# lmb-freiburg/hand3d

Hardware: NVIDIA H100
Metric: images/sec full pipeline 320x320 (higher is better)
Workload: dtype bf16 hi/lo split x3 MMA passes, fp32 accumulate (fp32 parity, 1e-3)

## Files before the change

### hand3d_b200/csrc/common.cuh

```cuda
#pragma once
#include <cuda_runtime.h>
#include <cuda_bf16.h>
#include <cuda_fp16.h>
#include <stdint.h>
#include <stdio.h>
#include <algorithm>
#include <cmath>
#include <string>

#include "../../include/hand3d_b200.h"

namespace h3d {

void set_error(const char* fmt, ...);
int cuda_fail(cudaError_t e, const char* what, const char* file, int line);

#define H3D_CUDA(expr)                                                     \
    do {                                                                   \
        cudaError_t _e = (expr);                                           \
        if (_e != cudaSuccess) return h3d::cuda_fail(_e, #expr, __FILE__, __LINE__); \
    } while (0)

#define H3D_CHECK_LAUNCH() H3D_CUDA(cudaGetLastError())

// ... 165 lines not shown
              int out_f, int leaky, int x_stride, cudaStream_t s);
int launch_concat_handside(const float* feat, const float* hand_side, float* out, int B, int feat_n, cudaStream_t s);
int launch_concat_handside_split(const float* feat, const float* hand_side, Split out, int B, int feat_n, int Kpad, Half16 t, cudaStream_t s);

int launch_conv_c3_tc(const float* x, const float* w, const float* bias, Split y, int Cs_total, int cs_off, int B, int H, int W, int leaky,
                      Half16 half, cudaStream_t s, int* err_flag = nullptr, const int* count = nullptr, const int* slots = nullptr);
struct TcConvPlan;
struct TcConvDesc {
    Split x;
    int Cin_total, Cin_pad;
    Split w;
    const float* bias;
    const float* w_scale = nullptr;
    int Cout, Cout_pad;
    Split y;
    int Cy_total, cy_off;
    float* yf;
    int Cyf_total, cyf_off;
    int B, H, W, k, leaky;
    int passes;
    float corr_scale = 0.f;
    Half16 half;
    int pool = 0;
    int* err_flag = nullptr;
    const int* count = nullptr;
};
struct TcTuning {
    int bn = 0;
    int chunk_kb = 0;
    int no_side_stream = 0, no_pool_fusion = 0, lift_direct = 0;
    int c3_ffma = 0;
    int no_seg_fusion = 0;
    int fc_chain = 1;
    int pdl = 1;
};
TcTuning& tc_tuning();
int tc_set_tuning(const char* key, int value);
struct FcLayerDesc {
    Split x; int x_stride, in_features;
    Split w; const float* bias; int out_features, out_pad;
    const float* w_scale = nullptr;
    Split y; int y_stride;
    float* yf; int yf_stride;
    int leaky;
};
struct FcChainDesc { FcLayerDesc layer[4]; int num_layers = 0; };
struct FcChainPlan;
FcChainPlan* fc_chain_plan_create(const FcChainDesc* chains, int num_chains, int B, Half16 half, const float* can, const float* uxyz,
                                  unsigned int* counter, int* err_flag);
void fc_chain_plan_destroy(FcChainPlan* p);
int fc_chain_launch(const FcChainPlan* p, const float* hand_side, float* rot, float* out, cudaStream_t s);
TcConvPlan* tc_conv_plan_create(const TcConvDesc& d, int* rc = nullptr);
void tc_conv_plan_destroy(TcConvPlan* p);
int tc_conv_launch(const TcConvPlan* p, cudaStream_t s);
int64_t tc_conv_flops(const TcConvPlan* p);
int tc_num_sms();
void tc_conv_geometry(int B, int H, int W, int Cout_pad, int pool, int passes, int out[4]);

int launch_pack_conv_w(const float* w_hwio, const float* bias, Split out, float* bias_pad, float* w_scale, int k, int Cin, int Cout,
                       int Cin_pad, int Cout_pad, bool dgrad, Half16 half, cudaStream_t s);
int conv_grad_prep_blocks(int64_t pixels, int64_t* pixels_per_block);
int launch_conv_grad_prep(const float* dy, const float* y, Split out, float* db_part, int B, int H, int W, int Cout, int Cout_pad,
                          int stride, int leaky, cudaStream_t s);
int launch_bias_grad_reduce(const float* db_part, int nblk, int Cout, int Cout_pad, float* db, cudaStream_t s);
struct WgradDesc {
    Split x;
// ... 39 lines not shown
```

### hand3d_b200/csrc/conv_wgmma.cu

```cuda
#include <cuda.h>

#include <algorithm>
#include <cstdlib>
#include <cstring>
#include <vector>

#include "common.cuh"
#include "split_fmt.cuh"
#include "wgmma_common.cuh"

namespace h3d {

namespace {

constexpr int BM = 128;
constexpr int BK = 64;
constexpr int kThreads = 384;
constexpr int kConsumerThreads = 256;
constexpr int A_TILE_BYTES = BM * BK * 2;
constexpr int STG_COLS = 64;
constexpr int STG_PITCH = STG_COLS + 1;
constexpr int STG_BYTES = BM * STG_PITCH * 4;
constexpr int kSmemBudget = 227 * 1024 - 2048 - STG_BYTES;

__host__ __device__ constexpr int stage_bytes(int BN, int PASSES) { return (PASSES >= 3 ? 2 : 1) * (A_TILE_BYTES + BN * BK * 2); }
__host__ __device__ constexpr int num_stages(int BN, int PASSES) {
    return kSmemBudget / stage_bytes(BN, PASSES) > 8 ? 8 : kSmemBudget / stage_bytes(BN, PASSES);
}
__host__ __device__ constexpr int smem_bytes(int BN, int PASSES) { return num_stages(BN, PASSES) * stage_bytes(BN, PASSES) + STG_BYTES + 2048; }

struct TcParams {
    const float* bias;
    uint16_t* y_hi; uint16_t* y_lo; uint8_t* y_l8; uint8_t* y_h8; int Cy_total, cy_off;
    float corr_scale;
    float* yf; int Cyf_total, cyf_off;
    int B, H, W, k, pad, cin_chunks;
    int TW, TH, TB, tiles_w, tiles_h, n_tiles, num_tiles;
    int n_valid;
    int pool;
    int chunk_kb;
    int leaky;
    int* err_flag;
    const float* w_scale;
    const int* count;
};

__device__ __forceinline__ int counted_images(const TcParams& p) { return p.count ? min(*p.count, p.B) : p.B; }
__device__ __forceinline__ int counted_tiles(const TcParams& p, int nb) {
    return p.count ? min(p.num_tiles, (nb + p.TB - 1) / p.TB * p.tiles_w * p.tiles_h * p.n_tiles) : p.num_tiles;
}

template <int PASSES, bool FP16, bool SMEM_SCALE = false>
__device__ __forceinline__ void epilogue_store32(const TcParams& p, const float* a, int64_t pix, int n, bool valid, const float* w_scale) {
    float f[32];
    const float4* bp = reinterpret_cast<const float4*>(p.bias + n);
#pragma unroll
    for (int q = 0; q < 8; ++q) {
        const float4 bv = __ldg(bp + q);
        if (PASSES == 4) {
            f[4 * q + 0] = fmaf(a[4 * q + 0], p.corr_scale, bv.x);
            f[4 * q + 1] = fmaf(a[4 * q + 1], p.corr_scale, bv.y);
            f[4 * q + 2] = fmaf(a[4 * q + 2], p.corr_scale, bv.z);
            f[4 * q + 3] = fmaf(a[4 * q + 3], p.corr_scale, bv.w);
        } else if (FP16) {
            const float4 sv = SMEM_SCALE ? reinterpret_cast<const float4*>(w_scale + n)[q] : __ldg(reinterpret_cast<const float4*>(w_scale + n) + q);
            f[4 * q + 0] = fmaf(a[4 * q + 0], sv.x, bv.x);
            f[4 * q + 1] = fmaf(a[4 * q + 1], sv.y, bv.y);
            f[4 * q + 2] = fmaf(a[4 * q + 2], sv.z, bv.z);
            f[4 * q + 3] = fmaf(a[4 * q + 3], sv.w, bv.w);
        } else {
            f[4 * q + 0] = a[4 * q + 0] + bv.x;
            f[4 * q + 1] = a[4 * q + 1] + bv.y;
            f[4 * q + 2] = a[4 * q + 2] + bv.z;
            f[4 * q + 3] = a[4 * q + 3] + bv.w;
        }
    }
    if (p.leaky) {
#pragma unroll
        for (int q = 0; q < 32; ++q) f[q] = fmaxf(f[q], kNegSlope * f[q]);
    }
    if (p.pool == 1) {
#pragma unroll
        for (int q = 0; q < 32; ++q) {
            f[q] = fmaxf(f[q], __shfl_xor_sync(0xFFFFFFFFu, f[q], 1));
            f[q] = fmaxf(f[q], __shfl_xor_sync(0xFFFFFFFFu, f[q], p.TW));
        }
    }
    if (!valid) return;
    if (n + 32 > p.n_valid) {
        const int cnt = p.n_valid - n;
        if (p.yf && cnt > 0) {
            float* dst = p.yf + pix * p.Cyf_total + p.cyf_off + n;
#pragma unroll
            for (int q = 0; q < 32; ++q)
                if (q < cnt) dst[q] = f[q];
        }
#pragma unroll
        for (int q = 0; q < 32; ++q)
            if (q >= cnt) f[q] = 0.f;
    } else if (p.yf) {
        if (((p.Cyf_total | p.cyf_off) & 3) == 0) {
            float4* dst = reinterpret_cast<float4*>(p.yf + pix * p.Cyf_total + p.cyf_off + n);
#pragma unroll
            for (int q = 0; q < 8; ++q) dst[q] = make_float4(f[4 * q], f[4 * q + 1], f[4 * q + 2], f[4 * q + 3]);
        } else {
            float* dst = p.yf + pix * p.Cyf_total + p.cyf_off + n;
#pragma unroll
            for (int q = 0; q < 32; ++q) dst[q] = f[q];
        }
    }
    if (p.y_hi) {
        const int64_t off = pix * p.Cy_total + p.cy_off + n;
        uint4* dh = reinterpret_cast<uint4*>(p.y_hi + off);
        uint4* dl = reinterpret_cast<uint4*>(p.y_lo + off);
#pragma unroll
        for (int g = 0; g < 4; ++g) {
            uint32_t hi[4], lo[4];
#pragma unroll
// ... 113 lines not shown
                for (int j = 0; j < 2; ++j) {
                    const uint64_t koff = (uint64_t)j * 2;
                    mma8<BN>(acc8, a_l8 + koff, b_h8 + koff, (uint32_t)((kb > kb0) | (j != 0)));
                    mma8<BN>(acc8, a_h8 + koff, b_l8 + koff, 1u);
                }
            }
            wgmma_commit();
            fence_regs<NR>(acc);
            fence_regs<NR8>(acc8);
            H3D_SKEW(SKEW_COMMIT, kb);
            wgmma_wait<1>();
            if (pend >= 0 && lane == 0) mbar_arrive(&r.empty[pend]);
            pend = r.stage;
            if (++r.stage == C::STAGES) { r.stage = 0; r.phase ^= 1; }
        }
        wgmma_wait<0>();
        if (lane == 0) mbar_arrive(&r.empty[pend]);
        fence_regs<NR>(acc);
        fence_regs<NR8>(acc8);
        if constexpr (PASSES == 4) {
#pragma unroll
            for (int i = 0; i < NR; ++i) acc[i] += acc8[i];
        }
        if (kb0 == 0) {
#pragma unroll
            for (int i = 0; i < NR; ++i) racc[i] = acc[i];
        } else {
#pragma unroll
            for (int i = 0; i < NR; ++i) racc[i] += acc[i];
        }
    }
}

template <int BN, int PASSES, bool FP16, class PixOf, bool SMEM_SCALE = false>
__device__ __forceinline__ void store_tile(const TcParams& p, const float* racc, float* stg, int ct, int n0, PixOf pix_of,
                                           const float* w_scale) {
    const int wg = ct >> 7, tt = ct & 127;
    const int r0 = wg * 64 + (tt >> 5) * 16 + ((tt & 31) >> 2);
    const int cq = 2 * (tt & 3);
    const int row = ct & 127, half = ct >> 7;
    int64_t pix; bool valid;
    pix_of(row, pix, valid);
#pragma unroll
    for (int rnd = 0; rnd < BN / STG_COLS; ++rnd) {
        H3D_SKEW(SKEW_EPILOGUE, 2 * rnd);
        named_bar_sync(1, kConsumerThreads);
#pragma unroll
        for (int j = 0; j < STG_COLS / 8; ++j) {
            const int jj = rnd * (STG_COLS / 8) + j, c = 8 * j + cq;
            stg[r0 * STG_PITCH + c] = racc[4 * jj];
            stg[r0 * STG_PITCH + c + 1] = racc[4 * jj + 1];
            stg[(r0 + 8) * STG_PITCH + c] = racc[4 * jj + 2];
            stg[(r0 + 8) * STG_PITCH + c + 1] = racc[4 * jj + 3];
        }
        named_bar_sync(1, kConsumerThreads);
        H3D_SKEW(SKEW_EPILOGUE, 2 * rnd + 1);
        float f[32];
#pragma unroll
        for (int q = 0; q < 32; ++q) f[q] = stg[row * STG_PITCH + half * 32 + q];
        epilogue_store32<PASSES, FP16, SMEM_SCALE>(p, f, pix, n0 + rnd * STG_COLS + half * 32, valid, w_scale);
    }
}

constexpr int kProducerRegs = 40, kConsumerRegs = 232;

template <int BN, int PASSES, bool FP16>
__global__ void __launch_bounds__(kThreads, 1)
conv_tc_kernel(const __grid_constant__ CUtensorMap map_x_hi, const __grid_constant__ CUtensorMap map_x_lo,
               const __grid_constant__ CUtensorMap map_w_hi, const __grid_constant__ CUtensorMap map_w_lo,
               const __grid_constant__ CUtensorMap map_x_h8, const __grid_constant__ CUtensorMap map_w_l8, const TcParams p) {
    using C = RingCfg<BN, PASSES>;
    static_assert(PASSES != 4 || FP16, "fp8-correction mode uses an fp16 main plane");
    static_assert(smem_bytes(BN, PASSES) <= 227 * 1024, "conv_tc_kernel: shared memory budget");

    extern __shared__ __align__(1024) uint8_t smem_raw[];
    uint8_t* smem = reinterpret_cast<uint8_t*>((reinterpret_cast<uintptr_t>(smem_raw) + 1023) & ~(uintptr_t)1023);
    float* stg = reinterpret_cast<float*>(smem + C::STAGES * C::STAGE_BYTES);
    uint64_t* bars = reinterpret_cast<uint64_t*>(smem + C::STAGES * C::STAGE_BYTES + STG_BYTES);
    Ring ring{smem, bars, bars + C::STAGES, 0, 0};

    const int warp = threadIdx.x >> 5, lane = threadIdx.x & 31;
    const int wg = __shfl_sync(0xFFFFFFFFu, (int)threadIdx.x / 128, 0);
    const int kblocks = p.k * p.k * p.cin_chunks;

    if (threadIdx.x == 0) {
        prefetch_tmap(&map_x_hi); prefetch_tmap(&map_w_hi);
        if (PASSES >= 3) { prefetch_tmap(&map_x_lo); prefetch_tmap(&map_w_lo); }
        if (PASSES == 4) { prefetch_tmap(&map_x_h8); prefetch_tmap(&map_w_l8); }
        for (int s = 0; s < C::STAGES; ++s) { mbar_init(&ring.full[s], 1); mbar_init(&ring.empty[s], kConsumerThreads / 32); }
        asm volatile("fence.mbarrier_init.release.cluster;" ::: "memory");
    }
    __syncthreads();
    pdl_launch_dependents();
    H3D_SKEW(SKEW_PDL_TAIL, 0);
    pdl_wait();
    const int nb = counted_images(p), num_tiles = counted_tiles(p, nb);

    if (wg == 0) {
        setmaxnreg_dec<kProducerRegs>();
        if (warp == 0) {
            for (int tile = blockIdx.x; tile < num_tiles; tile += gridDim.x) {
                const int nt = tile % p.n_tiles, mt = tile / p.n_tiles;
                const int tw = mt % p.tiles_w, th = (mt / p.tiles_w) % p.tiles_h, tb = mt / (p.tiles_w * p.tiles_h);
                const int w0 = tw * p.TW - p.pad, h0 = th * p.TH - p.pad, b0 = tb * p.TB, n0 = nt * BN;
                int kcol = 0;
                for (int kh = 0; kh < p.k; ++kh)
                    for (int kw = 0; kw < p.k; ++kw)
                        for (int cc = 0; cc < p.cin_chunks; ++cc, kcol += BK)
                            produce_kblock<BN, PASSES>(ring, &map_x_hi, &map_x_lo, &map_x_h8, &map_w_hi, &map_w_lo, &map_w_l8, cc * BK,
                                                       w0 + kw, h0 + kh, b0, kcol, n0, p.err_flag);
            }
        }
    } else {
        setmaxnreg_inc<kConsumerRegs>();
        const int ct = threadIdx.x - 128;
        float racc[BN / 2];
        for (int tile = blockIdx.x; tile < num_tiles; tile += gridDim.x) {
            const int nt = tile % p.n_tiles, mt = tile / p.n_tiles;
            const int tw = mt % p.tiles_w, th = (mt / p.tiles_w) % p.tiles_h, tb = mt / (p.tiles_w * p.tiles_h);
            mma_tile<BN, PASSES, FP16>(ring, kblocks, p.chunk_kb, racc, ct >> 7, lane, p.err_flag);
            store_tile<BN, PASSES, FP16>(p, racc, stg, ct, nt * BN, [&](int row, int64_t& pix, bool& valid) {
                const int w_l = row % p.TW, h_l = (row / p.TW) % p.TH, b_l = row / (p.TW * p.TH);
                const int w = tw * p.TW + w_l, h = th * p.TH + h_l, b = tb * p.TB + b_l;
                valid = (w < p.W) && (h < p.H) && (b < nb);
                pix = ((int64_t)b * p.H + h) * p.W + w;
                if (p.pool) {
                    const int par = p.pool == 2 ? 1 : 0;
                    valid = valid && ((w & 1) == par) && ((h & 1) == par);
                    pix = ((int64_t)b * (p.H >> 1) + (h >> 1)) * (p.W >> 1) + (w >> 1);
                }
            }, p.w_scale);
        }
    }
}

constexpr int C3_TW = 16, C3_TH = 8;
constexpr int C3T_THREADS = 256;
constexpr int C3T_B_BYTES = 128 * BK * 2;
constexpr int C3T_PW = C3_TW + 2, C3T_PH = C3_TH + 2;
constexpr int C3T_PATCH_FLOATS = C3T_PH * C3T_PW * 3;
constexpr int C3T_SMEM = C3T_B_BYTES + 2 * A_TILE_BYTES + STG_BYTES + C3T_PATCH_FLOATS * 4 + 64 * 4 + 1024 ;

template <bool FP16, bool COUNTED>
__global__ void __launch_bounds__(C3T_THREADS, 2)
conv_c3_tc_kernel(const float* __restrict__ x, const float* __restrict__ w, const TcParams p, const int* __restrict__ slots) {
    extern __shared__ __align__(1024) uint8_t smem_raw[];
    uint8_t* smem = reinterpret_cast<uint8_t*>((reinterpret_cast<uintptr_t>(smem_raw) + 1023) & ~(uintptr_t)1023);
    uint8_t* bsm = smem;
    uint8_t* asm_ = smem + C3T_B_BYTES;
    float* stg = reinterpret_cast<float*>(asm_ + 2 * A_TILE_BYTES);
    float* patch = stg + BM * STG_PITCH;
    float* w_scale = patch + C3T_PATCH_FLOATS;

    const int t = threadIdx.x, wg = t >> 7;
    if (t < 128) {
        const int co = t & 63;
        int sh = 0;
        if (FP16) {
            float mx = 0.f;
            for (int k = 0; k < 27; ++k) mx = fmaxf(mx, fabsf(__ldg(w + k * 64 + co)));
            sh = fp16_w_shift(mx);
            if (t < 64) w_scale[co] = ldexpf(1.f, -sh);
        }
        uint32_t pk[16];
// ... 223 lines not shown
                    box, estr, CU_TENSOR_MAP_INTERLEAVE_NONE, es == 2 ? CU_TENSOR_MAP_SWIZZLE_128B : CU_TENSOR_MAP_SWIZZLE_64B,
                    CU_TENSOR_MAP_L2_PROMOTION_L2_256B, CU_TENSOR_MAP_FLOAT_OOB_FILL_NONE);
    if (r != CUDA_SUCCESS) { set_error("cuTensorMapEncodeTiled(activations) failed: %d", (int)r); return false; }
    return true;
}

bool encode_w_map(CUtensorMap* m, const void* base, int Ktot, int Cout_pad, int BN, int es) {
    EncodeTiledFn fn = get_encode_fn();
    if (!fn) return false;
    cuuint64_t dims[2] = {(cuuint64_t)Ktot, (cuuint64_t)Cout_pad};
    cuuint64_t strides[1] = {(cuuint64_t)Ktot * es};
    cuuint32_t box[2] = {(cuuint32_t)BK, (cuuint32_t)BN};
    cuuint32_t estr[2] = {1, 1};
    CUresult r = fn(m, es == 2 ? CU_TENSOR_MAP_DATA_TYPE_UINT16 : CU_TENSOR_MAP_DATA_TYPE_UINT8, 2, const_cast<void*>(base), dims, strides,
                    box, estr, CU_TENSOR_MAP_INTERLEAVE_NONE, es == 2 ? CU_TENSOR_MAP_SWIZZLE_128B : CU_TENSOR_MAP_SWIZZLE_64B,
                    CU_TENSOR_MAP_L2_PROMOTION_L2_256B, CU_TENSOR_MAP_FLOAT_OOB_FILL_NONE);
    if (r != CUDA_SUCCESS) { set_error("cuTensorMapEncodeTiled(weights) failed: %d", (int)r); return false; }
    return true;
}

namespace {

void choose_tile(int B, int H, int W, int* TW, int* TH, int* TB, bool pool = false) {
    static const int cand[][3] = {{16, 8, 1}, {8, 16, 1}, {32, 4, 1}, {4, 32, 1}, {64, 2, 1}, {128, 1, 1}, {8, 8, 2},
                                  {16, 4, 2}, {4, 16, 2}, {8, 4, 4}, {4, 8, 4}, {4, 4, 8}, {8, 2, 8}, {2, 2, 32}, {1, 1, 128}};
    int64_t best = -1;
    for (auto& c : cand) {
        if (pool && !((c[0] % 2) == 0 && c[0] <= 16 && (c[1] % 2) == 0)) continue;
        const int64_t tiles = (int64_t)ceil_div(W, c[0]) * ceil_div(H, c[1]) * ceil_div(B, c[2]);
        if (best < 0 || tiles < best) { best = tiles; *TW = c[0]; *TH = c[1]; *TB = c[2]; }
    }
}

template <int BN, int PASSES, bool FP16>
int launch_inst(const TcConvPlan* pl, cudaStream_t s);

}

struct TcConvPlan {
    int device = 0;
    TcConvDesc d;
    CUtensorMap map_x_hi, map_x_lo, map_w_hi, map_w_lo, map_x_h8, map_w_l8;
    TcParams p;
    int BN, grid;
};

constexpr int kMaxDevices = 64;
static int current_device() { int dev = 0; if (cudaGetDevice(&dev) != cudaSuccess) { cudaGetLastError(); dev = 0; } return dev; }
int tc_num_sms() {
    static int n[kMaxDevices] = {};
    const int dev = current_device() % kMaxDevices;
    if (!n[dev]) {
        int v = 0;
        if (cudaDeviceGetAttribute(&v, cudaDevAttrMultiProcessorCount, dev) != cudaSuccess || v <= 0) { cudaGetLastError(); v = 132; }
        n[dev] = v;
    }
    return n[dev];
}
template <typename K>
static int smem_opt_in(K kernel, int bytes, bool* done ) {
    const int dev = current_device() % kMaxDevices;
    if (!done[dev]) {
        H3D_CUDA(cudaFuncSetAttribute(kernel, cudaFuncAttributeMaxDynamicSharedMemorySize, bytes));
        done[dev] = true;
    }
    return H3D_OK;
}

template <typename... KArgs, typename... Args>
static cudaError_t launch_pdl(void (*kernel)(KArgs...), dim3 grid, dim3 block, size_t smem, cudaStream_t s, Args&&... args) {
    cudaLaunchConfig_t cfg = {};
    cfg.gridDim = grid; cfg.blockDim = block; cfg.dynamicSmemBytes = smem; cfg.stream = s;
    cudaLaunchAttribute attr[1];
    attr[0].id = cudaLaunchAttributeProgrammaticStreamSerialization;
    attr[0].val.programmaticStreamSerializationAllowed = tc_tuning().pdl ? 1 : 0;
    cfg.attrs = attr; cfg.numAttrs = 1;
    return cudaLaunchKernelEx(&cfg, kernel, static_cast<KArgs>(args)...);
}

TcTuning& tc_tuning() {
    static TcTuning t = [] {
        TcTuning v;
        auto geti = [](const char* n, int d) { const char* e = getenv(n); return e ? atoi(e) : d; };
        v.bn = geti("H3D_TC_BN", 0);
        v.chunk_kb = geti("H3D_TC_CHUNK_KB", 0);
        v.no_side_stream = geti("H3D_NO_SIDE_STREAM", 0);
        v.no_pool_fusion = geti("H3D_NO_POOL_FUSION", 0);
        v.lift_direct = geti("H3D_LIFT_DIRECT", 0);
        v.c3_ffma = geti("H3D_C3_FFMA", 0);
        v.pdl = geti("H3D_PDL", 1);
        v.fc_chain = geti("H3D_FC_CHAIN", 1);
        v.no_seg_fusion = geti("H3D_NO_SEG_FUSION", 0);
        return v;
    }();
    return t;
}
#ifdef H3D_SKEW_BUILD
static std::vector<int (*)(const SkewCfg&)>& skew_uploaders() { static std::vector<int (*)(const SkewCfg&)> v; return v; }
static SkewCfg g_skew_host = {};
int skew_register(int (*upload)(const SkewCfg&)) { skew_uploaders().push_back(upload); return 0; }
int skew_set(const char* key, int value) {
    static const char* const sites[SKEW_SITES] = {"producer", "consumer", "commit", "epilogue", "cluster", "pdl_tail", "ticket"};
    const std::string k(key);
    if (k == "skew_reset") g_skew_host = SkewCfg{};
    else {
        int s = 0;
        while (s < SKEW_SITES && k.compare(0, 5 + strlen(sites[s]) + 1, std::string("skew_") + sites[s] + "_") != 0) ++s;
        const std::string f = s < SKEW_SITES ? k.substr(5 + strlen(sites[s]) + 1) : "";
        SkewSiteCfg* c = s < SKEW_SITES ? &g_skew_host.site[s] : nullptr;
        if (c && f == "ns" && value >= 0) c->ns = std::min((unsigned)value, kSkewMaxNs);
        else if (c && f == "role" && value >= 0 && value <= SKEW_RANK0 + 15) c->role = (unsigned)value;
        else if (c && f == "period" && value >= 0) c->period = (unsigned)value;
        else if (c && f == "seed") c->seed = (unsigned)value;
        else { set_error("h3d_set_tuning: bad skew key '%s' or value %d", key, value); return H3D_EINVAL; }
    }
    for (auto up : skew_uploaders()) H3D_CUDA((cudaError_t)up(g_skew_host));
    return H3D_OK;
}
#endif

int tc_set_tuning(const char* key, int value) {
    TcTuning& t = tc_tuning();
    const std::string k(key ? key : "");
    if (k == "tc_bn") t.bn = value;
    else if (k == "tc_chunk_kb") t.chunk_kb = value;
    else if (k == "no_side_stream") t.no_side_stream = value;
    else if (k == "no_pool_fusion") t.no_pool_fusion = value;
    else if (k == "lift_direct") t.lift_direct = value;
    else if (k == "c3_ffma") t.c3_ffma = value;
    else if (k == "pdl") t.pdl = value;
    else if (k == "fc_chain") t.fc_chain = value;
    else if (k == "no_seg_fusion") t.no_seg_fusion = value;
#ifdef H3D_SKEW_BUILD
    else if (k.compare(0, 5, "skew_") == 0) return skew_set(key, value);
#endif
    else { set_error("h3d_set_tuning: unknown key '%s'", k.c_str()); return H3D_EINVAL; }
    return H3D_OK;
}

namespace {
int choose_bn(int H, int W, int Cout_pad, int passes) {
    const TcTuning& tune = tc_tuning();
    int BN = Cout_pad % 128 == 0 ? 128 : 64;
    if ((int64_t)H * W <= 256) BN = 64;
    if ((tune.bn == 64 || tune.bn == 128) && Cout_pad % tune.bn == 0) BN = tune.bn;
    if (passes == 4) BN = 64;
    return BN;
}

template <int BN, int PASSES, bool FP16>
int launch_inst(const TcConvPlan* pl, cudaStream_t s) {
    constexpr int smem = smem_bytes(BN, PASSES);
    static bool attr[kMaxDevices] = {};
    if (int rc = smem_opt_in(conv_tc_kernel<BN, PASSES, FP16>, smem, attr)) return rc;
    H3D_CUDA(launch_pdl(conv_tc_kernel<BN, PASSES, FP16>, dim3(pl->grid), dim3(kThreads), smem, s, pl->map_x_hi, pl->map_x_lo, pl->map_w_hi,
                        pl->map_w_lo, pl->map_x_h8, pl->map_w_l8, pl->p));
    return H3D_OK;
}
}

TcConvPlan* tc_conv_plan_create(const TcConvDesc& d, int* rc) {
    int rc_local;
    if (!rc) rc = &rc_local;
    *rc = H3D_EINVAL;
    if (d.Cin_pad % BK != 0 || d.Cout_pad % 64 != 0 || (d.k != 1 && d.k != 3 && d.k != 5 && d.k != 7) || (d.passes != 1 && d.passes != 3 && d.passes != 4)) {
// ... 13 lines not shown
    }
    if (d.half == Half16::FP16 && d.passes != 4 && !d.w_scale) { set_error("tc_conv: fp16 weight planes need their per-channel scales"); return nullptr; }
    if (d.passes == 4 && d.y.hi && (!d.y.l8 || !d.y.h8)) { set_error("tc_conv: fp8-correction mode needs l8/h8 output planes"); return nullptr; }
    if (d.passes == 4 && d.y.hi && ((d.Cy_total % 16) || (d.cy_off % 16))) { set_error("tc_conv: fp8 planes need 16-channel aligned offsets"); return nullptr; }
    if (d.pool && ((d.H | d.W) & 1)) { set_error("tc_conv: fused max-pool / stride 2 needs even H and W"); return nullptr; }
    *rc = H3D_ECUDA;
    TcConvPlan* pl = new TcConvPlan();
    pl->d = d;
    const TcTuning& tune = tc_tuning();
    const int BN = choose_bn(d.H, d.W, d.Cout_pad, d.passes);
    int TW, TH, TB;
    choose_tile(d.B, d.H, d.W, &TW, &TH, &TB, d.pool == 1);
    pl->BN = BN;
    pl->device = current_device();
    TcParams& p = pl->p;
    p.bias = d.bias;
    p.y_hi = d.y.hi; p.y_lo = d.y.lo; p.y_l8 = d.y.l8; p.y_h8 = d.y.h8; p.Cy_total = d.Cy_total; p.cy_off = d.cy_off;
    p.corr_scale = d.corr_scale;
    p.yf = d.yf; p.Cyf_total = d.Cyf_total; p.cyf_off = d.cyf_off;
    p.B = d.B; p.H = d.H; p.W = d.W; p.k = d.k; p.pad = d.k / 2; p.cin_chunks = d.Cin_pad / BK;
    p.TW = TW; p.TH = TH; p.TB = TB;
    p.tiles_w = ceil_div(d.W, TW); p.tiles_h = ceil_div(d.H, TH);
    p.n_tiles = d.Cout_pad / BN;
    p.num_tiles = p.tiles_w * p.tiles_h * ceil_div(d.B, TB) * p.n_tiles;
    p.leaky = d.leaky;
    p.n_valid = d.Cout;
    p.pool = d.pool;
    p.err_flag = d.err_flag;
    p.w_scale = d.w_scale;
    p.count = d.count;
    p.chunk_kb = d.passes >= 3 ? 9 : 27;
    if (tune.chunk_kb > 0) p.chunk_kb = tune.chunk_kb;
    pl->grid = std::min(p.num_tiles, tc_num_sms());
    const int Ktot = d.k * d.k * d.Cin_pad;
    bool ok = encode_act_map(&pl->map_x_hi, d.x.hi, d.Cin_total, d.Cin_pad, d.W, d.H, d.B, TW, TH, TB) &&
              encode_w_map(&pl->map_w_hi, d.w.hi, Ktot, d.Cout_pad, BN);
    if (ok && d.passes == 3)
        ok = encode_act_map(&pl->map_x_lo, d.x.lo, d.Cin_total, d.Cin_pad, d.W, d.H, d.B, TW, TH, TB) &&
             encode_w_map(&pl->map_w_lo, d.w.lo, Ktot, d.Cout_pad, BN);
    if (ok && d.passes == 4)
        ok = encode_act_map(&pl->map_x_lo, d.x.l8, d.Cin_total, d.Cin_pad, d.W, d.H, d.B, TW, TH, TB, 1) &&
             encode_act_map(&pl->map_x_h8, d.x.h8, d.Cin_total, d.Cin_pad, d.W, d.H, d.B, TW, TH, TB, 1) &&
             encode_w_map(&pl->map_w_lo, d.w.h8, Ktot, d.Cout_pad, BN, 1) &&
             encode_w_map(&pl->map_w_l8, d.w.l8, Ktot, d.Cout_pad, BN, 1);
    if (ok && d.passes == 1) { pl->map_x_lo = pl->map_x_hi; pl->map_w_lo = pl->map_w_hi; }
    if (ok && d.passes != 4) { pl->map_x_h8 = pl->map_x_hi; pl->map_w_l8 = pl->map_w_hi; }
    if (!ok) { delete pl; return nullptr; }
    *rc = H3D_OK;
    return pl;
}

void tc_conv_plan_destroy(TcConvPlan* p) { delete p; }

void tc_conv_geometry(int B, int H, int W, int Cout_pad, int pool, int passes, int out[4]) {
    choose_tile(B, H, W, &out[0], &out[1], &out[2], pool == 1);
    out[3] = choose_bn(H, W, Cout_pad, passes);
}

int64_t tc_conv_flops(const TcConvPlan* p) {
    return 2ll * p->d.B * p->d.H * p->d.W * p->d.k * p->d.k * (int64_t)p->d.Cin_pad * p->d.Cout_pad;
}

int tc_conv_launch(const TcConvPlan* pl, cudaStream_t s) {
    const bool fp16 = pl->d.half == Half16::FP16;
    const int key = pl->BN * 10 + pl->d.passes;
#define CASE(BN_, P_)                                                                  \
    case BN_ * 10 + P_:                                                                \
        return fp16 ? launch_inst<BN_, P_, true>(pl, s) : launch_inst<BN_, P_, false>(pl, s);
    switch (key) {
        CASE(64, 1) CASE(64, 3) CASE(128, 1) CASE(128, 3)
        case 64 * 10 + 4: return launch_inst<64, 4, true>(pl, s);
// ... 87 lines not shown
```

### hand3d_b200/csrc/wgmma_common.cuh

```cuda
#pragma once
#include <cuda.h>

#include "common.cuh"
#include "skew.cuh"

namespace h3d {

namespace {

__device__ __forceinline__ uint32_t smem_u32(const void* p) { return (uint32_t)__cvta_generic_to_shared(p); }

__device__ __forceinline__ void mbar_init(uint64_t* bar, uint32_t count) {
    asm volatile("mbarrier.init.shared::cta.b64 [%0], %1;" ::"r"(smem_u32(bar)), "r"(count) : "memory");
}
__device__ __forceinline__ void mbar_expect_tx(uint64_t* bar, uint32_t bytes) {
    asm volatile("mbarrier.arrive.expect_tx.shared::cta.b64 _, [%0], %1;" ::"r"(smem_u32(bar)), "r"(bytes) : "memory");
}
__device__ __forceinline__ void mbar_arrive(uint64_t* bar) {
    asm volatile("mbarrier.arrive.shared::cta.b64 _, [%0];" ::"r"(smem_u32(bar)) : "memory");
}
constexpr uint32_t kTryWaitHintNs = 20000u;
__device__ __forceinline__ bool mbar_try_wait(uint64_t* bar, uint32_t parity) {
    uint32_t ok;
    asm volatile(
// ... 20 lines not shown
        : "memory");
}
__device__ __forceinline__ void tma_load_2d(const CUtensorMap* map, void* dst, uint64_t* bar, int c0, int c1) {
    asm volatile(
        "cp.async.bulk.tensor.2d.shared::cluster.global.mbarrier::complete_tx::bytes [%0], [%1, {%3, %4}], [%2];"
        ::"r"(smem_u32(dst)), "l"(reinterpret_cast<uint64_t>(map)), "r"(smem_u32(bar)), "r"(c0), "r"(c1)
        : "memory");
}
template <int N> __device__ __forceinline__ void setmaxnreg_dec() { asm volatile("setmaxnreg.dec.sync.aligned.u32 %0;" ::"n"(N)); }
template <int N> __device__ __forceinline__ void setmaxnreg_inc() { asm volatile("setmaxnreg.inc.sync.aligned.u32 %0;" ::"n"(N)); }
__device__ __forceinline__ void prefetch_tmap(const CUtensorMap* map) {
    asm volatile("prefetch.tensormap [%0];" ::"l"(reinterpret_cast<uint64_t>(map)) : "memory");
}

__device__ __forceinline__ void pdl_launch_dependents() { asm volatile("griddepcontrol.launch_dependents;" ::: "memory"); }
__device__ __forceinline__ void pdl_wait() { asm volatile("griddepcontrol.wait;" ::: "memory"); }

__device__ __forceinline__ bool elect_one() {
    uint32_t pred;
    asm volatile("{\n\t.reg .pred p;\n\telect.sync _|p, 0xffffffff;\n\tselp.u32 %0, 1, 0, p;\n\t}" : "=r"(pred));
    return pred != 0;
}
__device__ __forceinline__ void cluster_sync_all() {
    asm volatile("barrier.cluster.arrive.release.aligned;" ::: "memory");
    asm volatile("barrier.cluster.wait.acquire.aligned;" ::: "memory");
}
__device__ __forceinline__ uint32_t cluster_ctarank() { uint32_t r; asm volatile("mov.u32 %0, %%cluster_ctarank;" : "=r"(r)); return r; }
__device__ __forceinline__ void fence_proxy_async_smem() { asm volatile("fence.proxy.async.shared::cta;" ::: "memory"); }
__device__ __forceinline__ void named_bar_sync(int id, int threads) { asm volatile("bar.sync %0, %1;" ::"r"(id), "r"(threads) : "memory"); }
__device__ __forceinline__ uint32_t sw128_chunk(int r, int c) { return (uint32_t)(r * 128 + ((c ^ (r & 7)) << 4)); }

__device__ __forceinline__ uint64_t desc_sw128(uint32_t saddr) {
    return (uint64_t)((saddr & 0x3FFFFu) >> 4) | (1ull << 16) | (64ull << 32) | (1ull << 62);
}
__device__ __forceinline__ uint64_t desc_sw64(uint32_t saddr) {
    return (uint64_t)((saddr & 0x3FFFFu) >> 4) | (1ull << 16) | (32ull << 32) | (2ull << 62);
}
__device__ __forceinline__ void wgmma_fence() { asm volatile("wgmma.fence.sync.aligned;" ::: "memory"); }
__device__ __forceinline__ void wgmma_commit() { asm volatile("wgmma.commit_group.sync.aligned;" ::: "memory"); }
template <int N> __device__ __forceinline__ void wgmma_wait() { asm volatile("wgmma.wait_group.sync.aligned %0;" ::"n"(N) : "memory"); }
template <int NR> __device__ __forceinline__ void fence_regs(float* d) {
#pragma unroll
    for (int i = 0; i < NR; ++i) asm volatile("" : "+f"(d[i])::"memory");
}

__device__ __forceinline__ void wgmma_f16_n64(float* d, uint64_t a, uint64_t b, uint32_t scale_d) {
    asm volatile(
        "{\n\t.reg .pred p;\n\tsetp.ne.b32 p, %34, 0;\n\t"
        "wgmma.mma_async.sync.aligned.m64n64k16.f32.f16.f16 {%0, %1, %2, %3, %4, %5, %6, %7, %8, %9, %10, %11, %12, %13, %14, %15, %16, %17, %18, %19, %20, %21, %22, %23, %24, %25, %26, %27, %28, %29, %30, %31}, %32, %33, p, 1, 1, 0, 0;\n\t}"
        : "+f"(d[0]), "+f"(d[1]), "+f"(d[2]), "+f"(d[3]), "+f"(d[4]), "+f"(d[5]), "+f"(d[6]), "+f"(d[7]), "+f"(d[8]), "+f"(d[9]), "+f"(d[10]), "+f"(d[11]), "+f"(d[12]), "+f"(d[13]), "+f"(d[14]), "+f"(d[15]), "+f"(d[16]), "+f"(d[17]), "+f"(d[18]), "+f"(d[19]), "+f"(d[20]), "+f"(d[21]), "+f"(d[22]), "+f"(d[23]), "+f"(d[24]), "+f"(d[25]), "+f"(d[26]), "+f"(d[27]), "+f"(d[28]), "+f"(d[29]), "+f"(d[30]), "+f"(d[31])
        : "l"(a), "l"(b), "r"(scale_d));
}
__device__ __forceinline__ void wgmma_bf16_n64(float* d, uint64_t a, uint64_t b, uint32_t scale_d) {
    asm volatile(
        "{\n\t.reg .pred p;\n\tsetp.ne.b32 p, %34, 0;\n\t"
        "wgmma.mma_async.sync.aligned.m64n64k16.f32.bf16.bf16 {%0, %1, %2, %3, %4, %5, %6, %7, %8, %9, %10, %11, %12, %13, %14, %15, %16, %17, %18, %19, %20, %21, %22, %23, %24, %25, %26, %27, %28, %29, %30, %31}, %32, %33, p, 1, 1, 0, 0;\n\t}"
        : "+f"(d[0]), "+f"(d[1]), "+f"(d[2]), "+f"(d[3]), "+f"(d[4]), "+f"(d[5]), "+f"(d[6]), "+f"(d[7]), "+f"(d[8]), "+f"(d[9]), "+f"(d[10]), "+f"(d[11]), "+f"(d[12]), "+f"(d[13]), "+f"(d[14]), "+f"(d[15]), "+f"(d[16]), "+f"(d[17]), "+f"(d[18]), "+f"(d[19]), "+f"(d[20]), "+f"(d[21]), "+f"(d[22]), "+f"(d[23]), "+f"(d[24]), "+f"(d[25]), "+f"(d[26]), "+f"(d[27]), "+f"(d[28]), "+f"(d[29]), "+f"(d[30]), "+f"(d[31])
        : "l"(a), "l"(b), "r"(scale_d));
}
__device__ __forceinline__ void wgmma_e4m3_n64(float* d, uint64_t a, uint64_t b, uint32_t scale_d) {
    asm volatile(
        "{\n\t.reg .pred p;\n\tsetp.ne.b32 p, %34, 0;\n\t"
        "wgmma.mma_async.sync.aligned.m64n64k32.f32.e4m3.e4m3 {%0, %1, %2, %3, %4, %5, %6, %7, %8, %9, %10, %11, %12, %13, %14, %15, %16, %17, %18, %19, %20, %21, %22, %23, %24, %25, %26, %27, %28, %29, %30, %31}, %32, %33, p, 1, 1;\n\t}"
        : "+f"(d[0]), "+f"(d[1]), "+f"(d[2]), "+f"(d[3]), "+f"(d[4]), "+f"(d[5]), "+f"(d[6]), "+f"(d[7]), "+f"(d[8]), "+f"(d[9]), "+f"(d[10]), "+f"(d[11]), "+f"(d[12]), "+f"(d[13]), "+f"(d[14]), "+f"(d[15]), "+f"(d[16]), "+f"(d[17]), "+f"(d[18]), "+f"(d[19]), "+f"(d[20]), "+f"(d[21]), "+f"(d[22]), "+f"(d[23]), "+f"(d[24]), "+f"(d[25]), "+f"(d[26]), "+f"(d[27]), "+f"(d[28]), "+f"(d[29]), "+f"(d[30]), "+f"(d[31])
        : "l"(a), "l"(b), "r"(scale_d));
}
// ... 58 lines not shown
```

Measured before the change: 1240.

## Load halo activation tile once per channel chunk and reuse across 3x3 taps

For 3x3 convolutions with split passes 1 or 3, the producer now loads one (TW+2)x(TH+2) activation halo box per input-channel chunk instead of one shifted box per tap. The consumer addresses all nine taps inside that smem tile through offset wgmma descriptors with a custom stride. Weights stream through a separate ring. This cuts activation TMA traffic and redundant loads roughly ninefold, in exchange for a new barrier protocol, a changed pixel-to-row mapping, and a different pool shuffle lane.

After: 1249, median of 6. Within noise of the previous version (+0.8%).

```diff
diff --git a/hand3d_b200/csrc/common.cuh b/hand3d_b200/csrc/common.cuh
--- a/hand3d_b200/csrc/common.cuh
+++ b/hand3d_b200/csrc/common.cuh
@@ -221,6 +221,7 @@
     int c3_ffma = 0;
     int no_seg_fusion = 0;
     int fc_chain = 1;
+    int tc_halo = 1;
     int pdl = 1;
 };
 TcTuning& tc_tuning();
diff --git a/hand3d_b200/csrc/conv_wgmma.cu b/hand3d_b200/csrc/conv_wgmma.cu
--- a/hand3d_b200/csrc/conv_wgmma.cu
+++ b/hand3d_b200/csrc/conv_wgmma.cu
@@ -43,6 +43,9 @@
     int* err_flag;
     const float* w_scale;
     const int* count;
+    int halo;
+    int halo_wg_rows;
+    int pool_lane;
 };
 
 __device__ __forceinline__ int counted_images(const TcParams& p) { return p.count ? min(*p.count, p.B) : p.B; }
@@ -83,7 +86,7 @@
 #pragma unroll
         for (int q = 0; q < 32; ++q) {
             f[q] = fmaxf(f[q], __shfl_xor_sync(0xFFFFFFFFu, f[q], 1));
-            f[q] = fmaxf(f[q], __shfl_xor_sync(0xFFFFFFFFu, f[q], p.TW));
+            f[q] = fmaxf(f[q], __shfl_xor_sync(0xFFFFFFFFu, f[q], p.pool_lane));
         }
     }
     if (!valid) return;
@@ -263,6 +266,155 @@
     }
 }
 
+constexpr int kHaloMaxRows = 180;
+constexpr int kHaloMaxEntries = 16;
+
+__host__ __device__ constexpr int halo_plane_bytes(int rows) { return (rows * 128 + 1023) / 1024 * 1024; }
+__host__ __device__ constexpr int halo_entries(int BN, int PASSES, int rows) {
+    return (num_stages(BN, PASSES) * stage_bytes(BN, PASSES) - 2 * (PASSES >= 3 ? 2 : 1) * halo_plane_bytes(rows)) / (BN * BK * 2) >
+                   kHaloMaxEntries
+               ? kHaloMaxEntries
+               : (num_stages(BN, PASSES) * stage_bytes(BN, PASSES) - 2 * (PASSES >= 3 ? 2 : 1) * halo_plane_bytes(rows)) / (BN * BK * 2);
+}
+static_assert(halo_entries(128, 3, kHaloMaxRows) >= 6 && halo_entries(64, 3, kHaloMaxRows) >= 6, "halo ring: shared memory budget");
+static_assert(halo_entries(128, 1, kHaloMaxRows) >= 3 && halo_entries(64, 1, kHaloMaxRows) >= 3, "halo ring: shared memory budget");
+
+struct HaloRing {
+    uint8_t* base;
+    uint64_t* bars;
+    int plane_bytes, entries;
+    int hs, e;
+    uint32_t hph, bph;
+    __device__ uint64_t* hfull(int s) const { return bars + s; }
+    __device__ uint64_t* hempty(int s) const { return bars + 2 + s; }
+    __device__ uint64_t* bfull(int e_) const { return bars + 4 + e_; }
+    __device__ uint64_t* bempty(int e_) const { return bars + 4 + kHaloMaxEntries + e_; }
+};
+
+template <int BN, int PASSES>
+__device__ __forceinline__ HaloRing make_halo_ring(uint8_t* smem, uint64_t* bars, const TcParams& p) {
+    constexpr int planes = PASSES >= 3 ? 2 : 1;
+    HaloRing r;
+    r.base = smem;
+    r.bars = bars;
+    r.plane_bytes = halo_plane_bytes((p.TW + 2) * (p.TH + 2) * p.TB);
+    r.entries = min(kHaloMaxEntries, (num_stages(BN, PASSES) * stage_bytes(BN, PASSES) - 2 * planes * r.plane_bytes) / (BN * BK * 2));
+    r.hs = 0; r.e = 0; r.hph = 0; r.bph = 0;
+    return r;
+}
+
+template <int BN, int PASSES>
+__device__ __forceinline__ void produce_halo_tile(HaloRing& r, const CUtensorMap* x_hi, const CUtensorMap* x_lo, const CUtensorMap* w_hi,
+                                                  const CUtensorMap* w_lo, const TcParams& p, int w0, int h0, int b0, int n0) {
+    constexpr int planes = PASSES >= 3 ? 2 : 1;
+    const int box_bytes = (p.TW + 2) * (p.TH + 2) * p.TB * 128;
+    for (int cc = 0; cc < p.cin_chunks; ++cc) {
+        mbar_wait(r.hempty(r.hs), r.hph ^ 1, p.err_flag, 1);
+        H3D_SKEW(SKEW_PRODUCER, r.hs + 2 * r.hph);
+        if (elect_one()) {
+            uint8_t* slot = r.base + r.hs * (planes * r.plane_bytes);
+            mbar_expect_tx(r.hfull(r.hs), planes * box_bytes);
+            tma_load_4d(x_hi, slot, r.hfull(r.hs), cc * BK, w0, h0, b0);
+            if (PASSES == 3) tma_load_4d(x_lo, slot + r.plane_bytes, r.hfull(r.hs), cc * BK, w0, h0, b0);
+        }
+        __syncwarp();
+        if (++r.hs == 2) { r.hs = 0; r.hph ^= 1; }
+        for (int tap = 0; tap < 9; ++tap) {
+            const int kcol = (tap * p.cin_chunks + cc) * BK;
+#pragma unroll
+            for (int pl = 0; pl < planes; ++pl) {
+                mbar_wait(r.bempty(r.e), r.bph ^ 1, p.err_flag, 1);
+                H3D_SKEW(SKEW_PRODUCER, r.e + r.bph * r.entries);
+                if (elect_one()) {
+                    mbar_expect_tx(r.bfull(r.e), BN * BK * 2);
+                    tma_load_2d(pl ? w_lo : w_hi, r.base + 2 * (planes * r.plane_bytes) + r.e * (BN * BK * 2), r.bfull(r.e), kcol, n0);
+                }
+                __syncwarp();
+                if (++r.e == r.entries) { r.e = 0; r.bph ^= 1; }
+            }
+        }
+    }
+}
+
+template <int BN, int PASSES, bool FP16>
+__device__ __forceinline__ void mma_tile_halo(HaloRing& r, const TcParams& p, float* racc, int wg, int lane) {
+    constexpr int NR = BN / 2;
+    constexpr int planes = PASSES >= 3 ? 2 : 1;
+    const int kblocks = 9 * p.cin_chunks, chunk_kb = p.chunk_kb;
+    const int hw = p.TW + 2;
+    const uint32_t wg_off = (uint32_t)(wg * p.halo_wg_rows) * 128;
+    float acc[NR];
+#pragma unroll
+    for (int i = 0; i < NR; ++i) acc[i] = 0.f;
+    int tap = 0;
+    for (int kb0 = 0; kb0 < kblocks; kb0 += chunk_kb) {
+        const int kb1 = min(kblocks, kb0 + chunk_kb);
+        int pend = -1, pend_h = -1;
+        for (int kb = kb0; kb < kb1; ++kb) {
+            if (tap == 0) mbar_wait(r.hfull(r.hs), r.hph, p.err_flag, 3);
+            const int e0 = r.e;
+            mbar_wait(r.bfull(e0), r.bph, p.err_flag, 3);
+            int e1 = e0;
+            if (PASSES == 3) {
+                e1 = e0 + 1 == r.entries ? 0 : e0 + 1;
+                mbar_wait(r.bfull(e1), e1 ? r.bph : r.bph ^ 1, p.err_flag, 3);
+            }
+            H3D_SKEW(SKEW_CONSUMER, kb);
+            const int kh = tap / 3, kw = tap - 3 * kh;
+            const uint32_t slot = smem_u32(r.base + r.hs * (planes * r.plane_bytes)) + wg_off + (uint32_t)(kh * hw + kw) * 128;
+            const uint32_t sb = smem_u32(r.base + 2 * (planes * r.plane_bytes));
+            const uint64_t a_hi = desc_sw128_rows(slot, hw);
+            const uint64_t a_lo = desc_sw128_rows(slot + r.plane_bytes, hw);
+            const uint64_t b_hi = desc_sw128(sb + e0 * (BN * BK * 2));
+            const uint64_t b_lo = desc_sw128(sb + e1 * (BN * BK * 2));
+            fence_regs<NR>(acc);
+            wgmma_fence();
+#pragma unroll
+            for (int j = 0; j < BK / 16; ++j) {
+                const uint64_t koff = (uint64_t)j * 2;
+                mma16<BN, FP16>(acc, a_hi + koff, b_hi + koff, (uint32_t)((kb > kb0) | (j != 0)));
+                if (PASSES == 3) {
+                    mma16<BN, FP16>(acc, a_hi + koff, b_lo + koff, 1u);
+                    mma16<BN, FP16>(acc, a_lo + koff, b_hi + koff, 1u);
+                }
+            }
+            wgmma_commit();
+            fence_regs<NR>(acc);
+            H3D_SKEW(SKEW_COMMIT, kb);
+            wgmma_wait<1>();
+            if (lane == 0) {
+                if (pend >= 0) {
+                    mbar_arrive(r.bempty(pend));
+                    if (PASSES == 3) mbar_arrive(r.bempty(pend + 1 == r.entries ? 0 : pend + 1));
+                }
+                if (pend_h >= 0) mbar_arrive(r.hempty(pend_h));
+            }
+            pend = e0;
+            pend_h = tap == 8 ? r.hs : -1;
+            r.e = e0 + planes;
+            if (r.e >= r.entries) { r.e -= r.entries; r.bph ^= 1; }
+            if (++tap == 9) {
+                tap = 0;
+                if (++r.hs == 2) { r.hs = 0; r.hph ^= 1; }
+            }
+        }
+        wgmma_wait<0>();
+        if (lane == 0) {
+            mbar_arrive(r.bempty(pend));
+            if (PASSES == 3) mbar_arrive(r.bempty(pend + 1 == r.entries ? 0 : pend + 1));
+            if (pend_h >= 0) mbar_arrive(r.hempty(pend_h));
+        }
+        fence_regs<NR>(acc);
+        if (kb0 == 0) {
+#pragma unroll
+            for (int i = 0; i < NR; ++i) racc[i] = acc[i];
+        } else {
+#pragma unroll
+            for (int i = 0; i < NR; ++i) racc[i] += acc[i];
+        }
+    }
+}
+
 template <int BN, int PASSES, bool FP16, class PixOf, bool SMEM_SCALE = false>
 __device__ __forceinline__ void store_tile(const TcParams& p, const float* racc, float* stg, int ct, int n0, PixOf pix_of,
                                            const float* w_scale) {
@@ -309,6 +461,7 @@
     float* stg = reinterpret_cast<float*>(smem + C::STAGES * C::STAGE_BYTES);
     uint64_t* bars = reinterpret_cast<uint64_t*>(smem + C::STAGES * C::STAGE_BYTES + STG_BYTES);
     Ring ring{smem, bars, bars + C::STAGES, 0, 0};
+    static_assert(2 * C::STAGES <= 4 + 2 * kHaloMaxEntries && (4 + 2 * kHaloMaxEntries) * 8 <= 1024, "barrier space");
 
     const int warp = threadIdx.x >> 5, lane = threadIdx.x & 31;
     const int wg = __shfl_sync(0xFFFFFFFFu, (int)threadIdx.x / 128, 0);
@@ -318,7 +471,13 @@
         prefetch_tmap(&map_x_hi); prefetch_tmap(&map_w_hi);
         if (PASSES >= 3) { prefetch_tmap(&map_x_lo); prefetch_tmap(&map_w_lo); }
         if (PASSES == 4) { prefetch_tmap(&map_x_h8); prefetch_tmap(&map_w_l8); }
-        for (int s = 0; s < C::STAGES; ++s) { mbar_init(&ring.full[s], 1); mbar_init(&ring.empty[s], kConsumerThreads / 32); }
+        if (p.halo) {
+            const HaloRing halo = make_halo_ring<BN, PASSES>(smem, bars, p);
+            for (int s = 0; s < 2; ++s) { mbar_init(halo.hfull(s), 1); mbar_init(halo.hempty(s), kConsumerThreads / 32); }
+            for (int s = 0; s < halo.entries; ++s) { mbar_init(halo.bfull(s), 1); mbar_init(halo.bempty(s), kConsumerThreads / 32); }
+        } else {
+            for (int s = 0; s < C::STAGES; ++s) { mbar_init(&ring.full[s], 1); mbar_init(&ring.empty[s], kConsumerThreads / 32); }
+        }
         asm volatile("fence.mbarrier_init.release.cluster;" ::: "memory");
     }
     __syncthreads();
@@ -330,37 +489,56 @@
     if (wg == 0) {
         setmaxnreg_dec<kProducerRegs>();
         if (warp == 0) {
-            for (int tile = blockIdx.x; tile < num_tiles; tile += gridDim.x) {
-                const int nt = tile % p.n_tiles, mt = tile / p.n_tiles;
-                const int tw = mt % p.tiles_w, th = (mt / p.tiles_w) % p.tiles_h, tb = mt / (p.tiles_w * p.tiles_h);
-                const int w0 = tw * p.TW - p.pad, h0 = th * p.TH - p.pad, b0 = tb * p.TB, n0 = nt * BN;
-                int kcol = 0;
-                for (int kh = 0; kh < p.k; ++kh)
-                    for (int kw = 0; kw < p.k; ++kw)
-                        for (int cc = 0; cc < p.cin_chunks; ++cc, kcol += BK)
-                            produce_kblock<BN, PASSES>(ring, &map_x_hi, &map_x_lo, &map_x_h8, &map_w_hi, &map_w_lo, &map_w_l8, cc * BK,
-                                                       w0 + kw, h0 + kh, b0, kcol, n0, p.err_flag);
+            auto tiles = [&](auto&& produce) {
+                for (int tile = blockIdx.x; tile < num_tiles; tile += gridDim.x) {
+                    const int nt = tile % p.n_tiles, mt = tile / p.n_tiles;
+                    const int tw = mt % p.tiles_w, th = (mt / p.tiles_w) % p.tiles_h, tb = mt / (p.tiles_w * p.tiles_h);
+                    produce(tw * p.TW - p.pad, th * p.TH - p.pad, tb * p.TB, nt * BN);
+                }
+            };
+            if (PASSES != 4 && p.halo) {
+                HaloRing halo = make_halo_ring<BN, PASSES>(smem, bars, p);
+                tiles([&](int w0, int h0, int b0, int n0) {
+                    produce_halo_tile<BN, PASSES>(halo, &map_x_hi, &map_x_lo, &map_w_hi, &map_w_lo, p, w0, h0, b0, n0);
+                });
+            } else {
+                tiles([&](int w0, int h0, int b0, int n0) {
+                    for (int cc = 0; cc < p.cin_chunks; ++cc)
+                        for (int kh = 0; kh < p.k; ++kh)
+                            for (int kw = 0; kw < p.k; ++kw)
+                                produce_kblock<BN, PASSES>(ring, &map_x_hi, &map_x_lo, &map_x_h8, &map_w_hi, &map_w_lo, &map_w_l8, cc * BK,
+                                                           w0 + kw, h0 + kh, b0, ((kh * p.k + kw) * p.cin_chunks + cc) * BK, n0, p.err_flag);
+                });
             }
         }
     } else {
         setmaxnreg_inc<kConsumerRegs>();
         const int ct = threadIdx.x - 128;
         float racc[BN / 2];
-        for (int tile = blockIdx.x; tile < num_tiles; tile += gridDim.x) {
-            const int nt = tile % p.n_tiles, mt = tile / p.n_tiles;
-            const int tw = mt % p.tiles_w, th = (mt / p.tiles_w) % p.tiles_h, tb = mt / (p.tiles_w * p.tiles_h);
-            mma_tile<BN, PASSES, FP16>(ring, kblocks, p.chunk_kb, racc, ct >> 7, lane, p.err_flag);
-            store_tile<BN, PASSES, FP16>(p, racc, stg, ct, nt * BN, [&](int row, int64_t& pix, bool& valid) {
-                const int w_l = row % p.TW, h_l = (row / p.TW) % p.TH, b_l = row / (p.TW * p.TH);
-                const int w = tw * p.TW + w_l, h = th * p.TH + h_l, b = tb * p.TB + b_l;
-                valid = (w < p.W) && (h < p.H) && (b < nb);
-                pix = ((int64_t)b * p.H + h) * p.W + w;
-                if (p.pool) {
-                    const int par = p.pool == 2 ? 1 : 0;
-                    valid = valid && ((w & 1) == par) && ((h & 1) == par);
-                    pix = ((int64_t)b * (p.H >> 1) + (h >> 1)) * (p.W >> 1) + (w >> 1);
-                }
-            }, p.w_scale);
+        auto tiles = [&](auto&& mainloop) {
+            for (int tile = blockIdx.x; tile < num_tiles; tile += gridDim.x) {
+                const int nt = tile % p.n_tiles, mt = tile / p.n_tiles;
+                const int tw = mt % p.tiles_w, th = (mt / p.tiles_w) % p.tiles_h, tb = mt / (p.tiles_w * p.tiles_h);
+                mainloop();
+                store_tile<BN, PASSES, FP16>(p, racc, stg, ct, nt * BN, [&](int row, int64_t& pix, bool& valid) {
+                    int w_l = row % p.TW, h_l = (row / p.TW) % p.TH, b_l = row / (p.TW * p.TH);
+                    if (p.halo && p.TW == 16) { w_l = (row >> 6) * 8 + (row & 7); h_l = (row >> 3) & 7; }
+                    const int w = tw * p.TW + w_l, h = th * p.TH + h_l, b = tb * p.TB + b_l;
+                    valid = (w < p.W) && (h < p.H) && (b < nb);
+                    pix = ((int64_t)b * p.H + h) * p.W + w;
+                    if (p.pool) {
+                        const int par = p.pool == 2 ? 1 : 0;
+                        valid = valid && ((w & 1) == par) && ((h & 1) == par);
+                        pix = ((int64_t)b * (p.H >> 1) + (h >> 1)) * (p.W >> 1) + (w >> 1);
+                    }
+                }, p.w_scale);
+            }
+        };
+        if (PASSES != 4 && p.halo) {
+            HaloRing halo = make_halo_ring<BN, PASSES>(smem, bars, p);
+            tiles([&] { mma_tile_halo<BN, PASSES, FP16>(halo, p, racc, ct >> 7, lane); });
+        } else {
+            tiles([&] { mma_tile<BN, PASSES, FP16>(ring, kblocks, p.chunk_kb, racc, ct >> 7, lane, p.err_flag); });
         }
     }
 }
@@ -650,6 +828,12 @@
     }
 }
 
+int halo_wg_rows(int TW, int TH, int TB) {
+    if (TW == 16 && TH == 8 && TB == 1) return 8;
+    if (TW == 8 && TH == 16 && TB == 1) return 8 * (TW + 2);
+    return 0;
+}
+
 template <int BN, int PASSES, bool FP16>
 int launch_inst(const TcConvPlan* pl, cudaStream_t s);
 
@@ -709,6 +893,7 @@
         v.pdl = geti("H3D_PDL", 1);
         v.fc_chain = geti("H3D_FC_CHAIN", 1);
         v.no_seg_fusion = geti("H3D_NO_SEG_FUSION", 0);
+        v.tc_halo = geti("H3D_TC_HALO", 1);
         return v;
     }();
     return t;
@@ -749,6 +934,7 @@
     else if (k == "pdl") t.pdl = value;
     else if (k == "fc_chain") t.fc_chain = value;
     else if (k == "no_seg_fusion") t.no_seg_fusion = value;
+    else if (k == "tc_halo") t.tc_halo = value;
 #ifdef H3D_SKEW_BUILD
     else if (k.compare(0, 5, "skew_") == 0) return skew_set(key, value);
 #endif
@@ -828,11 +1014,15 @@
     p.chunk_kb = d.passes >= 3 ? 9 : 27;
     if (tune.chunk_kb > 0) p.chunk_kb = tune.chunk_kb;
     pl->grid = std::min(p.num_tiles, tc_num_sms());
+    p.halo_wg_rows = d.k == 3 && d.passes != 4 && tune.tc_halo ? halo_wg_rows(TW, TH, TB) : 0;
+    p.halo = p.halo_wg_rows > 0;
+    p.pool_lane = p.halo ? 8 : TW;
+    const int BW = p.halo ? TW + 2 : TW, BH = p.halo ? TH + 2 : TH;
     const int Ktot = d.k * d.k * d.Cin_pad;
-    bool ok = encode_act_map(&pl->map_x_hi, d.x.hi, d.Cin_total, d.Cin_pad, d.W, d.H, d.B, TW, TH, TB) &&
+    bool ok = encode_act_map(&pl->map_x_hi, d.x.hi, d.Cin_total, d.Cin_pad, d.W, d.H, d.B, BW, BH, TB) &&
               encode_w_map(&pl->map_w_hi, d.w.hi, Ktot, d.Cout_pad, BN);
     if (ok && d.passes == 3)
-        ok = encode_act_map(&pl->map_x_lo, d.x.lo, d.Cin_total, d.Cin_pad, d.W, d.H, d.B, TW, TH, TB) &&
+        ok = encode_act_map(&pl->map_x_lo, d.x.lo, d.Cin_total, d.Cin_pad, d.W, d.H, d.B, BW, BH, TB) &&
              encode_w_map(&pl->map_w_lo, d.w.lo, Ktot, d.Cout_pad, BN);
     if (ok && d.passes == 4)
         ok = encode_act_map(&pl->map_x_lo, d.x.l8, d.Cin_total, d.Cin_pad, d.W, d.H, d.B, TW, TH, TB, 1) &&
diff --git a/hand3d_b200/csrc/wgmma_common.cuh b/hand3d_b200/csrc/wgmma_common.cuh
--- a/hand3d_b200/csrc/wgmma_common.cuh
+++ b/hand3d_b200/csrc/wgmma_common.cuh
@@ -76,6 +76,9 @@
 
 __device__ __forceinline__ uint64_t desc_sw128(uint32_t saddr) {
     return (uint64_t)((saddr & 0x3FFFFu) >> 4) | (1ull << 16) | (64ull << 32) | (1ull << 62);
+}
+__device__ __forceinline__ uint64_t desc_sw128_rows(uint32_t saddr, uint32_t sbo_rows) {
+    return (uint64_t)((saddr & 0x3FFFFu) >> 4) | (1ull << 16) | ((uint64_t)(sbo_rows * 8) << 32) | (1ull << 62);
 }
 __device__ __forceinline__ uint64_t desc_sw64(uint32_t saddr) {
     return (uint64_t)((saddr & 0x3FFFFu) >> 4) | (1ull << 16) | (32ull << 32) | (2ull << 62);
```
